# Fanchuana/OPUS-PLLM

Hardware: AMD Instinct MI355X
Metric: proteins_per_sec (higher is better)
Workload: dtype f16; 1 GPU; OPUS-PLLM-llama3_8b shape: batch 64/GPU, 512-residue proteins, 89-id prompt (+8 protein tokens = 96 positions), 32 new tokens, greedy (BASELINE configs[3] per-GPU shard: batch 512 over 8 GPUs); batch_per_gpu=64, residues=512, parallelism=replicas x1 (batch-sharded), all-gather of ids

## Files before the change

### opus-pllm_amd/csrc/api.cpp

```cpp
#include "../../include/opus_pllm.h"
#include "common.h"

#include <cmath>
#include <cstdarg>
#include <cstdio>
#include <cstdlib>
#include <cstring>
#include <algorithm>
#include <atomic>
#include <map>
#include <string>
#include <vector>

using namespace opus;

static thread_local char g_err[512] = "";
static int fail(int code, const char *fmt, ...) {
    va_list ap;
    va_start(ap, fmt);
    vsnprintf(g_err, sizeof(g_err), fmt, ap);
    va_end(ap);
    return code;
}
#define HIPC(expr)                                                                                   \
// ... 1023 lines not shown
        KL(KC_OTHER, 4.0 * M * F, launch_relu_h(c->d_act, (int64_t)M * F, s));
    }
    OPC(gemm(c, s, c->d_act, F, L.w2, M, H, F, L.b2, EPI_NONE, x, x, H, 1));
    return OPUS_OK;
}

static int lm_head_opt(opus_ctx *c, hipStream_t s, int B) {
    const opus_config &g = c->cfg;
    KL(KC_NORM, 6.0 * B * g.dec_dim, launch_layernorm(c->d_xl, c->dec_lnfw, c->dec_lnfb, g.dec_rms_eps, B, g.dec_dim, c->d_xln, nullptr, s));
    return gemm(c, s, c->d_xln, g.dec_dim, c->lm_head, B, g.dec_vocab, g.dec_dim, nullptr, EPI_NONE, nullptr, c->d_logits,
                g.dec_vocab, 1);
}

static int prefill_opt(opus_ctx *c, hipStream_t s, const half_t *embeds, const uint8_t *mask, int B, int T, bool all_rows,
                       const ContRows *cont) {
    const opus_config &g = c->cfg;
    const int H = g.dec_dim, M = B * T;
    HIPC(hipMemsetAsync(c->d_cnt, 0, HANDOFF_ERR * sizeof(int32_t), s));
    if (!cont) KL(KC_OTHER, 1.0 * M, launch_mask_to_kstart(mask, B, T, c->d_kstart, s));
    KL(KC_OTHER, 6.0 * M * H, launch_h2f(embeds, c->d_x, (int64_t)M * H, s));
    KL(KC_OTHER, 10.0 * M * H, launch_add_pos(c->d_x, c->dec_pos, cont ? cont->nkst : c->d_kstart, nullptr, 0, B, T, H, g.dec_max_pos + 1, s));
    for (int l = 0; l < g.dec_layers; ++l) OPC(opt_layer(c, s, c->dec[l], l, c->d_x, c->d_xn, M, B, T, false, cont));
    if (all_rows) return OPUS_OK;
    KL(KC_OTHER, 8.0 * B * H, launch_take_last(c->d_x, B, T, H, c->d_xl, s));
    OPC(lm_head_opt(c, s, B));
    OPC(reset_step(c, s, T));
    c->cur_B = B;
    c->cur_T = T;
    c->prefilled = true;
    return OPUS_OK;
}

static int decode_step_opt(opus_ctx *c, hipStream_t s) {
    const opus_config &g = c->cfg;
    const int B = c->cur_B, T = c->cur_T, H = g.dec_dim;
    KL(KC_OTHER, 10.0 * B * H, launch_add_pos(c->d_xl, c->dec_pos, c->d_kstart, c->d_step, -1, B, 1, H, g.dec_max_pos + 1, s));
    for (int l = 0; l < g.dec_layers; ++l) OPC(opt_layer(c, s, c->dec[l], l, c->d_xl, c->d_xln, B, B, T, true));
    OPC(lm_head_opt(c, s, B));
    KL(KC_OTHER, 8.0, launch_step_advance(c->d_step, s));
    return OPUS_OK;
}

static int prefill(opus_ctx *c, hipStream_t s, const half_t *embeds, const uint8_t *mask, int B, int T, bool all_rows = false,
                   const ContRows *cont = nullptr) {
    c->phase = cont ? PH_SCORE : PH_PREFILL;
    if (cont) {
        all_rows = true;
    } else {
        new_epoch(c);
        if (all_rows) {
            c->prefilled = false;
            c->cur_B = 0;
        }
    }
    if (c->cfg.dec_arch == 1) return prefill_opt(c, s, embeds, mask, B, T, all_rows, cont);
    const opus_config &g = c->cfg;
    const int H = g.dec_dim, F = g.dec_ffn, nh = g.dec_heads, nkv = g.dec_kv_heads, hd = g.dec_head_dim;
    const int QKV = (nh + 2 * nkv) * hd, QD = nh * hd;
    const int M = B * T;
    HIPC(hipMemsetAsync(c->d_cnt, 0, HANDOFF_ERR * sizeof(int32_t), s));
    if (!cont) KL(KC_OTHER, 1.0 * M, launch_mask_to_kstart(mask, B, T, c->d_kstart, s));
    KL(KC_OTHER, 6.0 * M * H, launch_h2f(embeds, c->d_x, (int64_t)M * H, s));
    static const bool no_ln_env = getenv("OPUS_NO_LN_FUSION") != nullptr;
    const bool no_ln_fusion = no_ln_env || g_knobs.no_ln_fusion;
    const bool qkv_pp = !no_ln_fusion && (H & 255) == 0 && (QKV & 255) == 0 && gemm_goes_pp(M, QKV);
    const bool gu_pp = !no_ln_fusion && (H & 255) == 0 && (F & 127) == 0 && gemm_goes_pp(M, 2 * F);
    bool have_stat = false, last_rows_done = false;
    auto finalize = [&]() -> int {
        KL(KC_NORM, 8.0 * M * (H / 64) + 8.0 * M, launch_ln_finalize(c->d_part, M, H / 64, H, g.dec_rms_eps, 1, c->d_stat, s));
        return OPUS_OK;
    };
    for (int l = 0; l < g.dec_layers; ++l) {
        const DecLayer &L = c->dec[l];
        if (have_stat && qkv_pp) {
            c->rq_ln_stat = c->d_stat;
            OPC(gemm(c, s, c->d_xn, H, L.wqkv, M, QKV, H, L.bqkv, EPI_NONE, nullptr, c->d_qkv, QKV, 0));
        } else {
            OPC(gemm_norm(c, s, c->d_x, g.dec_rms_eps, c->d_xn, L.wqkv, M, QKV, H, EPI_NONE, c->d_qkv, QKV, 0, L.bqkv));
        }
        if (cont) {
            KL(KC_OTHER, 4.0 * M * QKV, launch_dec_rope_cache(c->d_qkv, c->cs_dec, cont->nkst, B, T, nh, nkv, hd, nullptr, nullptr, 0, 0, s));
            OPC(attn_prefix(c, s, *cont, l, M));
        } else {
            KL(KC_OTHER, 4.0 * M * QKV,
               launch_dec_rope_cache(c->d_qkv, c->cs_dec, c->d_kstart, B, T, nh, nkv, hd, c->kc + l * c->cache_sl,
                                     c->vc + l * c->cache_sl, c->cache_sb, c->cache_sh, s));
            AttnParams a;
            a.Q = c->d_qkv; a.K = c->d_qkv + QD; a.V = c->d_qkv + QD + nkv * hd;
            a.q_sb = a.k_sb = a.v_sb = (int64_t)T * QKV;
            a.q_st = a.k_st = a.v_st = QKV;
            a.O = c->d_ctx; a.o_sb = (int64_t)T * QD; a.o_st = QD;
            a.kstart = c->d_kstart; a.kend = nullptr;
            a.B = B; a.T = T; a.heads = nh; a.group = nh / nkv; a.head_dim = hd; a.causal = 1;
            a.scale = 1.0f / sqrtf((float)hd);
            KLF(KC_ATTN_PREFILL, 2.0 * M * (QKV + QD), 2.0 * B * (double)T * T * QD, launch_attn_prefill(a, s));
        }
        if (l + 1 == g.dec_layers && T > 1 && !all_rows && !g_knobs.misc[7]) {
            half_t *ctx_last = c->d_qkv;
            KL(KC_OTHER, 4.0 * B * QD, launch_take_last(reinterpret_cast<const float *>(c->d_ctx), B, T, QD / 2, reinterpret_cast<float *>(ctx_last), s));
            KL(KC_OTHER, 8.0 * B * H, launch_take_last(c->d_x, B, T, H, c->d_xl, s));
            if (fuse_rows() && B <= 96) c->rq_xh = c->d_xln;
            OPC(gemm(c, s, ctx_last, QD, L.wo, B, H, QD, nullptr, EPI_NONE, c->d_xl, c->d_xl, H, 1));
            c->xh_src = c->rq_done ? c->d_xl : nullptr;
            OPC(gemm_norm(c, s, c->d_xl, g.dec_rms_eps, c->d_xln, L.wgu, B, 2 * F, H, EPI_SILU_GU16, c->d_act, F, 0));
            if (fuse_rows() && B <= 96) c->rq_xh = c->d_xln;
            OPC(gemm(c, s, c->d_act, F, L.wd, B, H, F, nullptr, EPI_NONE, c->d_xl, c->d_xl, H, 1));
            c->xh_src = c->rq_done ? c->d_xl : nullptr;
            c->xln_tiled = false;
            last_rows_done = true;
            break;
        }
        if (gu_pp) { c->rq_ln_part = c->d_part; c->rq_ln_xh = c->d_xn; }
        else if (fuse_rows() && M <= 96) c->rq_xh = c->d_xn;
        OPC(gemm(c, s, c->d_ctx, QD, L.wo, M, H, QD, nullptr, EPI_NONE, c->d_x, c->d_x, H, 1));
        c->xh_src = c->rq_done ? c->d_x : nullptr;
        have_stat = c->rq_ln_done != 0;
        if (have_stat) {
            OPC(finalize());
            c->rq_ln_stat = c->d_stat;
            OPC(gemm(c, s, c->d_xn, H, L.wgu, M, 2 * F, H, nullptr, EPI_SILU_GU16, nullptr, c->d_act, F, 0));
        } else {
            OPC(gemm_norm(c, s, c->d_x, g.dec_rms_eps, c->d_xn, L.wgu, M, 2 * F, H, EPI_SILU_GU16, c->d_act, F, 0));
        }
        if (qkv_pp && l + 1 < g.dec_layers) { c->rq_ln_part = c->d_part; c->rq_ln_xh = c->d_xn; }
        OPC(gemm(c, s, c->d_act, F, L.wd, M, H, F, nullptr, EPI_NONE, c->d_x, c->d_x, H, 1));
        have_stat = c->rq_ln_done != 0;
        if (have_stat) OPC(finalize());
    }
    if (all_rows) {
        c->xh_src = nullptr;
        return OPUS_OK;
    }
    if (!last_rows_done) {
        KL(KC_OTHER, 8.0 * B * H, launch_take_last(c->d_x, B, T, H, c->d_xl, s));
        c->xh_src = nullptr;
    }
    OPC(lm_head(c, s, B));
    OPC(reset_step(c, s, T));
    c->cur_B = B;
    c->cur_T = T;
    c->prefilled = true;
    return OPUS_OK;
}

static int decode_step(opus_ctx *c, hipStream_t s, const int32_t *d_tok) {
    c->phase = PH_DECODE;
    const opus_config &g = c->cfg;
    const int B = c->cur_B, T = c->cur_T;
    const int H = g.dec_dim, F = g.dec_ffn, nh = g.dec_heads, nkv = g.dec_kv_heads, hd = g.dec_head_dim;
    const int QKV = (nh + 2 * nkv) * hd, QD = nh * hd;
    const int ctx_cap = g.max_prompt + g.max_new_tokens;
    const bool rowscale = g.dec_arch == 0 && fuse_rows() && B > SKINNY_MAX_M && B <= MID_MAX_M && (H & 255) == 0;
    const bool qkv_tiled = rowscale && gemm_stream_would(B, QKV, H, 1, 1, 1, c->gemm_ws_bytes);
    const bool wo_tiled = rowscale && gemm_stream_would(B, H, QD, 0, 1, 0, c->gemm_ws_bytes);
    const bool down_tiled = rowscale && (F & 63) == 0 && gemm_stream_would(B, H, F, 0, 1, 0, c->gemm_ws_bytes);
    KL(KC_OTHER, 6.0 * B * H, launch_embed_tokens(d_tok, c->dec_emb, B, H, g.dec_vocab, c->d_xl, rowscale ? c->d_xln : nullptr,
                                                  rowscale ? c->d_ssq : nullptr, qkv_tiled ? 1 : 0, c->cs_dec, c->d_kstart, c->d_step, -1,
                                                  hd / 2, c->cs_row, c->d_cnt, HANDOFF_ERR, s));
    c->xln_tiled = qkv_tiled;
    c->xh_src = rowscale ? c->d_xl : nullptr;
    if (rowscale) c->ssq_nblk = H >> 8;
    if (g.dec_arch == 1) return decode_step_opt(c, s);
    for (int l = 0; l < g.dec_layers; ++l) {
        const DecLayer &L = c->dec[l];
        if (rowscale && c->xh_src == c->d_xl) {
            c->xh_src = nullptr;
            c->rq_force_wide = 1;
            c->rq_slab_only = 1;
            c->use_row_scale = true;
            c->row_eps = g.dec_rms_eps;
            c->rq_a_tiled = c->xln_tiled ? 1 : 0;
            OPC(gemm(c, s, c->d_xln, H, L.wqkv, B, QKV, H, L.bqkv, EPI_NONE, nullptr, c->d_qkv, QKV, 0));
            OPC(attn_decode(c, s, l, B, T, c->rq_ks > 1 ? c->rq_ks : 0, L.bqkv, wo_tiled ? 1 : 0));
        } else {
            OPC(gemm_norm(c, s, c->d_xl, g.dec_rms_eps, c->d_xln, L.wqkv, B, QKV, H, EPI_NONE, c->d_qkv, QKV, 0, L.bqkv));
            OPC(attn_decode(c, s, l, B, T, 0, nullptr, wo_tiled ? 1 : 0));
        }
        c->xln_tiled = false;
// ... 1169 lines not shown
    new_epoch(c);
    const int nkv = g.dec_kv_heads, hd = g.dec_head_dim, T0 = c->cur_T;
    for (int l = 0; l < g.dec_layers; ++l) {
        half_t *kc = c->kc + l * c->cache_sl, *vc = c->vc + l * c->cache_sl;
        KL(KC_OTHER, 8.0 * R * nkv * hd * T0, launch_kv_gather_rows(kc, c->kv_tmp, d_src_rows, R, (int64_t)row, nkv, c->cache_sh, c->d_step, T0, hd, 0, s));
        HIPC(launch_kv_gather_rows(vc, c->kv_tmp + layer, d_src_rows, R, (int64_t)row, nkv, c->cache_sh, c->d_step, T0, hd, 0, s));
        HIPC(launch_kv_gather_rows(kc, c->kv_tmp, d_src_rows, R, (int64_t)row, nkv, c->cache_sh, c->d_step, T0, hd, 1, s));
        HIPC(launch_kv_gather_rows(vc, c->kv_tmp + layer, d_src_rows, R, (int64_t)row, nkv, c->cache_sh, c->d_step, T0, hd, 1, s));
    }
    return OPUS_OK;
}

extern "C" int opus_last_logits(opus_ctx *c, float *d_out, int32_t B, void *stream) {
    if (!c || !d_out) return fail(OPUS_EBADARG, "last_logits: null pointer");
    if (!c->prefilled) return fail(OPUS_ESTATE, "last_logits before prefill");
    if (B < 1 || B > c->cur_B) return fail(OPUS_ESHAPE, "last_logits: B=%d but the last prefill had %d rows", B, c->cur_B);
    HIPC(hipSetDevice(c->device));
    HIPC(hipMemcpyAsync(d_out, c->d_logits, (size_t)B * c->cfg.dec_vocab * sizeof(float), hipMemcpyDeviceToDevice, (hipStream_t)stream));
    return OPUS_OK;
}

extern "C" int opus_debug_attention(opus_ctx *c, const void *Q, const void *K, const void *V, void *O,
                                    const int32_t *kstart, const int32_t *kend, int32_t B, int32_t T, int32_t heads,
                                    int32_t group, int32_t hd, int32_t causal, float scale, void *stream) {
    if (!c || !Q || !K || !V || !O) return fail(OPUS_EBADARG, "debug_attention: null pointer");
    if (B < 1 || T < 1 || heads < 1 || group < 1 || heads % group) return fail(OPUS_ESHAPE, "debug_attention: shape");
    HIPC(hipSetDevice(c->device));
    hipStream_t s = (hipStream_t)stream;
    AttnParams a;
    const int kvh = heads / group;
    a.Q = (const half_t *)Q; a.K = (const half_t *)K; a.V = (const half_t *)V; a.O = (half_t *)O;
    a.q_st = (int64_t)heads * hd; a.q_sb = a.q_st * T;
    a.k_st = a.v_st = (int64_t)kvh * hd; a.k_sb = a.v_sb = a.k_st * T;
    a.o_st = a.q_st; a.o_sb = a.q_sb;
    a.kstart = kstart; a.kend = kend; a.B = B; a.T = T; a.heads = heads; a.group = group; a.head_dim = hd;
    a.causal = causal; a.scale = scale;
    KLF(KC_ATTN_PREFILL, 2.0 * B * T * hd * (2.0 * heads + 2.0 * kvh), (causal ? 2.0 : 4.0) * B * (double)T * T * heads * hd,
        launch_attn_prefill(a, s));
    return OPUS_OK;
}

extern "C" int opus_debug_attn_decode(opus_ctx *c, const void *d_qkv, const void *d_k_hist, const void *d_v_hist,
                                      const int32_t *d_kstart, int32_t B, int32_t T0, int32_t step, void *d_out, void *d_k_new,
                                      void *d_v_new, void *stream) {
    if (!c || !d_qkv || !d_kstart || !d_out) return fail(OPUS_EBADARG, "debug_attn_decode: null pointer");
    const opus_config &g = c->cfg;
    const int L = T0 + step, nkv = g.dec_kv_heads, hd = g.dec_head_dim;
    if (B < 1 || B > g.max_batch || T0 < 1 || T0 > g.max_prompt || step < 0 || step >= g.max_new_tokens)
        return fail(OPUS_ESHAPE, "debug_attn_decode: B=%d T0=%d step=%d exceed the context (%d, %d, %d)", B, T0, step, g.max_batch,
                    g.max_prompt, g.max_new_tokens);
    if (L > 0 && (!d_k_hist || !d_v_hist)) return fail(OPUS_EBADARG, "debug_attn_decode: history is null");
    HIPC(hipSetDevice(c->device));
    hipStream_t s = (hipStream_t)stream;
    const size_t pitch = (size_t)c->cache_sh * sizeof(half_t), roww = (size_t)L * hd * sizeof(half_t);
    HIPC(hipMemcpy2DAsync(c->kc, pitch, d_k_hist, roww, roww, (size_t)B * nkv, hipMemcpyDeviceToDevice, s));
    HIPC(hipMemcpy2DAsync(c->vc, pitch, d_v_hist, roww, roww, (size_t)B * nkv, hipMemcpyDeviceToDevice, s));
    HIPC(hipMemcpyAsync(c->d_kstart, d_kstart, (size_t)B * sizeof(int32_t), hipMemcpyDeviceToDevice, s));
    OPC(reset_step(c, s, T0, step));
    HIPC(launch_embed_tokens(c->d_next, nullptr, B, 0, 1, c->d_xl, nullptr, nullptr, 0, c->cs_dec, c->d_kstart, c->d_step, -1, hd / 2,
                             c->cs_row, nullptr, 0, s));
    AttnDecodeParams a;
    a.qkv = (const half_t *)d_qkv; a.slabs = nullptr; a.ks = 0; a.slab_stride = 0; a.row_ssq = nullptr; a.row_nblk = 0; a.eps = 0.f; a.K = 0;
    a.bias = nullptr;
    a.cs_row = c->cs_row; a.kstart = c->d_kstart; a.step = c->d_step; a.T0 = -1; a.nh = g.dec_heads; a.nkv = nkv;
    a.kc = c->kc; a.vc = c->vc; a.cache_sb = c->cache_sb; a.cache_sh = c->cache_sh;
    a.ctx_cap = g.max_prompt + g.max_new_tokens; a.scale = 1.0f / sqrtf((float)hd); a.out = (half_t *)d_out; a.out_tiled = 0;
    c->phase = PH_DECODE;
    KL(KC_ATTN_DECODE, 4.0 * B * nkv * hd * (L + 1), launch_attn_decode(a, B, hd, s));
    const size_t one = (size_t)hd * sizeof(half_t);
    if (d_k_new) HIPC(hipMemcpy2DAsync(d_k_new, one, c->kc + (size_t)L * hd, pitch, one, (size_t)B * nkv, hipMemcpyDeviceToDevice, s));
    if (d_v_new) HIPC(hipMemcpy2DAsync(d_v_new, one, c->vc + (size_t)L * hd, pitch, one, (size_t)B * nkv, hipMemcpyDeviceToDevice, s));
    c->prefilled = false;
    new_epoch(c);
    return OPUS_OK;
}

extern "C" int opus_debug_knob(opus_ctx *c, const char *name, int32_t value) {
    if (!name) return fail(OPUS_EBADARG, "debug_knob: null name");
    if (c) drop_graphs(c);
    if (!strcmp(name, "no_stream")) g_knobs.no_stream = value;
    else if (!strcmp(name, "debug_a_tiled")) g_knobs.debug_a_tiled = value;
    else if (!strcmp(name, "no_ln_fusion")) g_knobs.no_ln_fusion = value;
    else if (!strcmp(name, "enc_full_last_layer")) g_knobs.enc_full_last_layer = value;
    else if (!strcmp(name, "poison_handoff")) {
        if (!c) return fail(OPUS_EBADARG, "poison_handoff needs a context");
        std::vector<int32_t> h(HANDOFF_ERR, 0);
        if (value) for (int i = 0; i < HANDOFF_ERR; ++i) h[i] = i < 512 ? value : ((i & 1) ? 0 : 1);
        HIPC(hipSetDevice(c->device));
        HIPC(hipDeviceSynchronize());
        HIPC(hipMemcpy(c->d_cnt, h.data(), h.size() * sizeof(int32_t), hipMemcpyHostToDevice));
    }
    else if (!strcmp(name, "pp_gm")) { if (value < 1 || value > 64) return fail(OPUS_EBADARG, "pp_gm out of range"); g_knobs.pp_gm = value; }
    else if (!strncmp(name, "misc", 4) && name[4] >= '0' && name[4] <= '7' && !name[5]) g_knobs.misc[name[4] - '0'] = value;
    else return fail(OPUS_EBADARG, "debug_knob: unknown knob '%s'", name);
    return OPUS_OK;
}

extern "C" int64_t opus_stat(opus_ctx *c, const char *name) {
    if (!c || !name) return -1;
    if (!strcmp(name, "graph_instantiations")) return c->graph_instantiations;
    if (!strcmp(name, "graph_replays")) return c->graph_replays;
    if (!strcmp(name, "graphs_cached")) return (int64_t)c->graphs.size();
    if (!strcmp(name, "decode_steps")) return c->decode_steps;
    return -1;
}

extern "C" int opus_timing_enable(opus_ctx *c, int32_t on) {
    if (!c) return fail(OPUS_EBADARG, "ctx is null");
    c->timing = on != 0;
    return OPUS_OK;
}
extern "C" int opus_timing_reset(opus_ctx *c) {
    if (!c) return fail(OPUS_EBADARG, "ctx is null");
    HIPC(hipDeviceSynchronize());
    timing_clear(c);
    return OPUS_OK;
}
static const char *kclass_names[KC_COUNT] = {"gemm_skinny", "gemm_mid", "gemm_wide", "gemm_ring", "gemm_pp", "gemm_tile", "splitk_reduce",
                                            "attn_prefill", "attn_decode", "norm", "other", "gemm_stream", "contact", "constraint", "logitproc",
                                            "xent"};
static const char *phase_names[PH_COUNT] = {"encode", "project", "splice", "prefill", "decode", "other", "score"};

extern "C" int opus_timing_get(opus_ctx *c, const char *kernel_class, const char *phase, double *ms, int64_t *launches,
                               double *bytes, double *flops) {
    if (!c || !kernel_class || !phase || !ms || !launches || !bytes || !flops) return fail(OPUS_EBADARG, "null argument");
    int k = -1, ph = -1;
    const bool any_k = !strcmp(kernel_class, "*"), any_p = !strcmp(phase, "*");
    for (int i = 0; i < KC_COUNT; ++i) if (!strcmp(kclass_names[i], kernel_class)) k = i;
    for (int i = 0; i < PH_COUNT; ++i) if (!strcmp(phase_names[i], phase)) ph = i;
    if (k < 0 && !any_k) return fail(OPUS_EBADARG, "unknown kernel class '%s'", kernel_class);
    if (ph < 0 && !any_p) return fail(OPUS_EBADARG, "unknown phase '%s'", phase);
    HIPC(hipDeviceSynchronize());
    double t = 0, b = 0, f = 0;
    int64_t n = 0;
    for (auto &r : c->recs) {
        if ((!any_k && r.klass != k) || (!any_p && r.phase != ph)) continue;
        float e = 0;
        HIPC(hipEventElapsedTime(&e, r.e0, r.e1));
        t += e;
        b += r.bytes;
        f += r.flops;
        ++n;
    }
    *ms = t;
    *launches = n;
    *bytes = b;
    *flops = f;
    return OPUS_OK;
}

extern "C" int opus_timing_names(char *buf, int32_t cap) {
    if (!buf || cap < 1) return fail(OPUS_EBADARG, "null buffer");
    std::string out;
    for (int i = 0; i < KC_COUNT; ++i) { out += kclass_names[i]; out += i + 1 < KC_COUNT ? "," : ";"; }
    for (int i = 0; i < PH_COUNT; ++i) { out += phase_names[i]; if (i + 1 < PH_COUNT) out += ","; }
    if ((int)out.size() + 1 > cap) return fail(OPUS_ESHAPE, "buffer too small (%zu needed)", out.size() + 1);
    memcpy(buf, out.c_str(), out.size() + 1);
    return OPUS_OK;
}
```

### opus-pllm_amd/csrc/attn_prefill.hip

```cpp
#include "common.h"
#include <type_traits>

namespace opus {

constexpr int KB = 64;

template <int HDP>
__device__ __forceinline__ int kswz(int row, int chunk) {
    if (HDP == 128) return chunk ^ (row & 15);
    if (HDP == 64) return chunk ^ ((row >> 1) & 7);
    return chunk;
}
template <int HD>
__device__ __forceinline__ int vswz(int row) {
    if (HD == 128) return (row & 7) << 1;
    if (HD == 64) return ((row >> 1) & 3) << 1;
    if (HD == 32) return ((row >> 2) & 1) << 1;
    return 0;
}

typedef float f2 __attribute__((ext_vector_type(2)));
__device__ __forceinline__ float max3(float a, float b, float c) {
    float r;
    asm("v_max3_f32 %0, %1, %2, %3" : "=v"(r) : "v"(a), "v"(b), "v"(c));
    return r;
}
__device__ __forceinline__ float xor16_max(float x) {
    float a = x, b = x, r;
    asm volatile("s_nop 1\n\tv_permlane16_swap_b32 %0, %1" : "+v"(a), "+v"(b));
    asm("v_max_f32 %0, %1, %2" : "=v"(r) : "v"(a), "v"(b));
    return r;
}
__device__ __forceinline__ void xor32_pair(float x, float &a, float &b) {
    a = x;
    b = x;
    asm volatile("s_nop 1\n\tv_permlane32_swap_b32 %0, %1" : "+v"(a), "+v"(b));
}

typedef short s4v __attribute__((ext_vector_type(4)));
typedef short s8v __attribute__((ext_vector_type(8)));

template <int HD, bool CAUSAL, int QT>
__global__ __launch_bounds__(256) void attn_prefill_kernel(AttnParams p) {
    constexpr int QW = 16 * QT, QB = 4 * QW;
    constexpr int HDP = HD < 32 ? 32 : HD;
    constexpr int KS = HDP / 32;
    constexpr int NO = HD / 16;
    constexpr int CH = HDP / 8;
    constexpr int VC = HD / 8;
    __shared__ __attribute__((aligned(16))) half_t sK[2][KB * HDP];
    __shared__ __attribute__((aligned(16))) half_t sV[2][KB * HD];

    const int tid = threadIdx.x, lane = tid & 63;
    const int wave = __builtin_amdgcn_readfirstlane(tid >> 6);
    const int g = lane >> 4, li = lane & 15;
    const int qtrim = (p.q_trim && p.cu) ? 1 : 0;
    const int nqb = (p.T - 2 * qtrim + QB - 1) / QB;
    const int id = blockIdx.x, slot = id >> 3;
    const int bh = (slot / nqb) * 8 + (id & 7);
    if (bh >= p.B * p.heads) return;
    const int b = bh / p.heads, h = bh % p.heads, hk = h / p.group;
    const int q0 = (slot % nqb) * QB + qtrim, qw = q0 + wave * QW;
    int T = p.T, Tq = p.T;
    int64_t qb_off = (int64_t)b * p.q_sb, kb_off = (int64_t)b * p.k_sb, vb_off = (int64_t)b * p.v_sb, ob_off = (int64_t)b * p.o_sb;
    if (p.cu) {
        const int r0 = p.cu[b];
        T = p.cu[b + 1] - r0;
        Tq = T - qtrim;
        if (q0 >= Tq) return;
        qb_off = (int64_t)r0 * p.q_st; kb_off = (int64_t)r0 * p.k_st; vb_off = (int64_t)r0 * p.v_st; ob_off = (int64_t)r0 * p.o_st;
    }
    const int kstart = (p.kstart && !p.cu) ? p.kstart[b] : 0;
    const int kend = (p.kend && !p.cu) ? p.kend[b] : T;

    const half_t *Qb = p.Q + qb_off + (int64_t)h * HD;
    const half_t *Kb = p.K + kb_off + (int64_t)hk * HD;
    const half_t *Vb = p.V + vb_off + (int64_t)hk * HD;

    h8 qf[QT][KS];
#pragma unroll
    for (int t = 0; t < QT; ++t) {
        int qr = qw + 16 * t + li;
        qr = qr < Tq ? qr : Tq - 1;
        const half_t *src = Qb + (int64_t)qr * p.q_st;
#pragma unroll
        for (int s = 0; s < KS; ++s) {
            const int d = 32 * s + 8 * g;
            qf[t][s] = d < HD ? *reinterpret_cast<const h8 *>(src + d) : h8{0, 0, 0, 0, 0, 0, 0, 0};
        }
    }
    f4 o[QT][NO];
    float mrow[QT], lrow[QT];
#pragma unroll
    for (int t = 0; t < QT; ++t) {
        mrow[t] = -INFINITY;
        lrow[t] = 0.f;
#pragma unroll
        for (int n = 0; n < NO; ++n) o[t][n] = f4{0.f, 0.f, 0.f, 0.f};
    }

    int k_lo = kstart / KB * KB;
    int k_hi = kend;
    if (CAUSAL) {
        const int last_q = (q0 + QB - 1 < T - 1 ? q0 + QB - 1 : T - 1);
        k_hi = k_hi < last_q + 1 ? k_hi : last_q + 1;
    }
    const float sc = p.scale * 1.4426950408889634f;
    const bool wave_live = qw < Tq;

    constexpr int KL = KB * CH / 256;
    constexpr int VN = KB * VC;
    constexpr int VL = VN >= 256 ? VN / 256 : 1;
    static_assert(KL >= 1, "tile too small for 256 threads");
    h8 kreg[KL], vreg[VL];
    const __amdgpu_buffer_rsrc_t krs = __builtin_amdgcn_make_buffer_rsrc((void *)Kb, 0, (int)(((int64_t)(T - 1) * p.k_st + HD) * 2), 0x00020000);
    const __amdgpu_buffer_rsrc_t vrs = __builtin_amdgcn_make_buffer_rsrc((void *)Vb, 0, (int)(((int64_t)(T - 1) * p.v_st + HD) * 2), 0x00020000);
    int koff[KL], voff[VL];
#pragma unroll
    for (int u = 0; u < KL; ++u) {
        const int i = tid + 256 * u, r = i / CH, c = i % CH;
        koff[u] = c * 8 < HD ? (int)((r * p.k_st + c * 8) * 2) : 0x7ffffff0;
    }
#pragma unroll
    for (int u = 0; u < VL; ++u) {
        const int i = tid + 256 * u, r = i / VC, c = i % VC;
        voff[u] = i < VN ? (int)((r * p.v_st + c * 8) * 2) : 0x7ffffff0;
    }
    auto load_tile = [&](int kt) {
        const int kb = kt * (int)p.k_st * 2, vb = kt * (int)p.v_st * 2;
#pragma unroll
        for (int u = 0; u < KL; ++u) kreg[u] = __builtin_bit_cast(h8, __builtin_amdgcn_raw_buffer_load_b128(krs, koff[u] + kb, 0, 0));
#pragma unroll
        for (int u = 0; u < VL; ++u) vreg[u] = __builtin_bit_cast(h8, __builtin_amdgcn_raw_buffer_load_b128(vrs, voff[u] + vb, 0, 0));
    };
    auto store_tile = [&](int buf) {
#pragma unroll
        for (int u = 0; u < KL; ++u) {
            const int i = tid + 256 * u, r = i / CH, c = i % CH;
            *reinterpret_cast<h8 *>(&sK[buf][r * HDP + kswz<HDP>(r, c) * 8]) = kreg[u];
        }
#pragma unroll
        for (int u = 0; u < VL; ++u) {
            const int i = tid + 256 * u, r = i / VC, c = i % VC;
            if (i < VN) *reinterpret_cast<h8 *>(&sV[buf][r * HD + (c ^ vswz<HD>(r)) * 8]) = vreg[u];
        }
    };

    if (k_lo < k_hi) {
        load_tile(k_lo);
        store_tile(0);
        if (k_lo + KB < k_hi) load_tile(k_lo + KB);
    }
    __syncthreads();
    auto tile_body = [&](auto nsub_tag, int kt, int buf) {
        {
            constexpr int NSUB = decltype(nsub_tag)::value, NJ = (NSUB + 1) / 2;
            const half_t *tK = sK[buf], *tV = sV[buf];
            f4 s[QT][4];
#pragma unroll
            for (int n = 0; n < NSUB; ++n) {
                const int r = 16 * n + li;
                h8 kf[KS];
#pragma unroll
                for (int ks = 0; ks < KS; ++ks) kf[ks] = *reinterpret_cast<const h8 *>(tK + r * HDP + kswz<HDP>(r, 4 * ks + g) * 8);
#pragma unroll
                for (int t = 0; t < QT; ++t) {
                    s[t][n] = f4{0.f, 0.f, 0.f, 0.f};
#pragma unroll
                    for (int ks = 0; ks < KS; ++ks) s[t][n] = mfma16(kf[ks], qf[t][ks], s[t][n]);
                }
            }
            const bool interior = kt >= kstart && kt + KB <= kend && (!CAUSAL || kt + KB - 1 <= qw);
            if (__builtin_expect(!interior, 0)) {
#pragma unroll
                for (int t = 0; t < QT; ++t) {
                    const int qi = qw + 16 * t + li;
#pragma unroll
                    for (int n = 0; n < NSUB; ++n)
#pragma unroll
                        for (int r = 0; r < 4; ++r) {
                            const int kj = kt + 16 * n + 4 * g + r;
                            bool vis = kj >= kstart && kj < kend;
                            if (CAUSAL) vis = vis && kj <= qi;
                            s[t][n][r] = vis ? s[t][n][r] : -INFINITY;
                        }
                }
            }
            h8 pf[QT][2];
#pragma unroll
            for (int t = 0; t < QT; ++t) {
                float mx = fmaxf(fmaxf(s[t][0][0], s[t][0][1]), fmaxf(s[t][0][2], s[t][0][3]));
#pragma unroll
                for (int n = 1; n < NSUB; ++n) mx = fmaxf(fmaxf(mx, fmaxf(s[t][n][0], s[t][n][1])), fmaxf(s[t][n][2], s[t][n][3]));
                float ma, mb;
                mx = xor16_max(mx);
                xor32_pair(mx, ma, mb);
                const float mnew = max3(mrow[t], ma, mb);
                const float msafe = mnew == -INFINITY ? 0.f : mnew;
                const float msc = msafe * sc;
                if (!__all(mnew == mrow[t])) {
                    const float alpha = __builtin_amdgcn_exp2f((mrow[t] - msafe) * sc);
                    lrow[t] *= alpha;
#pragma unroll
                    for (int n = 0; n < NO; ++n) o[t][n] *= alpha;
                    mrow[t] = mnew;
                }
                const f2 sc2 = f2{sc, sc}, msc2 = f2{msc, msc};
                f2 rs2 = f2{0.f, 0.f};
#pragma unroll
                for (int n = 0; n < NSUB; ++n)
#pragma unroll
                    for (int r = 0; r < 4; r += 2) {
                        const f2 a = f2{s[t][n][r], s[t][n][r + 1]} * sc2 - msc2;
                        const f2 e = f2{__builtin_amdgcn_exp2f(a[0]), __builtin_amdgcn_exp2f(a[1])};
                        s[t][n][r] = e[0];
                        s[t][n][r + 1] = e[1];
                        rs2 += e;
                    }
                lrow[t] += rs2[0] + rs2[1];
#pragma unroll
                for (int j = 0; j < NJ; ++j) {
                    const bool two = 2 * j + 1 < NSUB;
                    pf[t][j] = h8{(half_t)s[t][2 * j][0], (half_t)s[t][2 * j][1], (half_t)s[t][2 * j][2], (half_t)s[t][2 * j][3],
                                  two ? (half_t)s[t][two ? 2 * j + 1 : 0][0] : (half_t)0.f, two ? (half_t)s[t][two ? 2 * j + 1 : 0][1] : (half_t)0.f,
                                  two ? (half_t)s[t][two ? 2 * j + 1 : 0][2] : (half_t)0.f, two ? (half_t)s[t][two ? 2 * j + 1 : 0][3] : (half_t)0.f};
                }
            }
#pragma unroll
            for (int n = 0; n < NO; ++n)
#pragma unroll
                for (int j = 0; j < NJ; ++j) {
                    const int r0 = 16 * (2 * j) + 4 * g + (li >> 2), r1 = r0 + 16;
                    const int cc = 2 * n + ((li & 3) >> 1), off = (li & 1) * 4;
                    const s4v lo = __builtin_amdgcn_ds_read_tr16_b64_v4i16(
                        (__attribute__((address_space(3))) s4v *)(tV + r0 * HD + (cc ^ vswz<HD>(r0)) * 8 + off));
                    const s4v hi = __builtin_amdgcn_ds_read_tr16_b64_v4i16(
                        (__attribute__((address_space(3))) s4v *)(tV + r1 * HD + (cc ^ vswz<HD>(r1)) * 8 + off));
                    const s8v both = s8v{lo[0], lo[1], lo[2], lo[3], hi[0], hi[1], hi[2], hi[3]};
                    const h8 vf = __builtin_bit_cast(h8, both);
#pragma unroll
                    for (int t = 0; t < QT; ++t) o[t][n] = mfma16(vf, pf[t][j], o[t][n]);
                }
        }
    };
    auto run = [&](auto live_tag) {
        constexpr bool LIVE = decltype(live_tag)::value;
        int kt = k_lo, buf = 0;
        for (; k_hi - kt > 32; kt += KB, buf ^= 1) {
            if constexpr (LIVE) tile_body(std::integral_constant<int, 4>{}, kt, buf);
            if (kt + KB < k_hi) {
                store_tile(buf ^ 1);
                if (kt + 2 * KB < k_hi) load_tile(kt + 2 * KB);
            }
            __syncthreads();
        }
        if constexpr (LIVE) {
            if (kt < k_hi) {
                if (k_hi - kt > 16) tile_body(std::integral_constant<int, 2>{}, kt, buf);
                else tile_body(std::integral_constant<int, 1>{}, kt, buf);
            }
        }
    };
    if (wave_live) run(std::true_type{});
    else run(std::false_type{});

    if (!wave_live) return;
#pragma unroll
    for (int t = 0; t < QT; ++t) {
        float l = lrow[t];
        l += __shfl_xor(l, 16, 64);
        l += __shfl_xor(l, 32, 64);
        const int qi = qw + 16 * t + li;
        if (qi >= Tq) continue;
        const float inv = l > 0.f ? 1.0f / l : 0.f;
        half_t *dst = p.O + ob_off + (int64_t)qi * p.o_st + (int64_t)h * HD;
#pragma unroll
        for (int n = 0; n < NO; ++n)
            *reinterpret_cast<h4 *>(dst + 16 * n + 4 * g) =
                h4{(half_t)(o[t][n][0] * inv), (half_t)(o[t][n][1] * inv), (half_t)(o[t][n][2] * inv), (half_t)(o[t][n][3] * inv)};
    }
}

template <int HD, int QT>
static hipError_t launch_qt(const AttnParams &p, hipStream_t s) {
    const int nqb = cdiv(p.T - ((p.q_trim && p.cu) ? 2 : 0), 64 * QT);
    dim3 grid(((p.B * p.heads + 7) / 8) * 8 * nqb);
    if (p.causal) OPUS_LAUNCH(KC_ATTN_PREFILL, (attn_prefill_kernel<HD, true, QT>), grid, dim3(256), 0, s, p);
    else OPUS_LAUNCH(KC_ATTN_PREFILL, (attn_prefill_kernel<HD, false, QT>), grid, dim3(256), 0, s, p);
    return hipGetLastError();
}
template <int HD>
static hipError_t launch_hd(const AttnParams &p, hipStream_t s) {
    bool one = !(HD <= 64 && (int64_t)p.B * p.heads * cdiv(p.T, 128) >= 512);
    if (g_knobs.misc[3]) one = !one;
    return one ? launch_qt<HD, 1>(p, s) : launch_qt<HD, 2>(p, s);
}

hipError_t launch_attn_prefill(const AttnParams &p, hipStream_t s) {
    if (p.T <= 0 || p.B <= 0) return hipErrorInvalidValue;
    if ((p.o_st & 3) || (p.o_sb & 3) || (p.q_st & 7) || (p.k_st & 7) || (p.v_st & 7) || (p.q_sb & 7) || (p.k_sb & 7) || (p.v_sb & 7))
        return hipErrorInvalidValue;
    if ((int64_t)p.T * (p.k_st > p.v_st ? p.k_st : p.v_st) * 2 >= (1ll << 31)) return hipErrorInvalidValue;
    switch (p.head_dim) {
        case 16: return launch_hd<16>(p, s);
        case 32: return launch_hd<32>(p, s);
        case 64: return launch_hd<64>(p, s);
        case 128: return launch_hd<128>(p, s);
    }
    return hipErrorInvalidValue;
}

}
```

### opus-pllm_amd/csrc/common.h

```cpp
#pragma once
#include <hip/hip_runtime.h>
#include <hip/hip_ext.h>
#include <stdint.h>

namespace opus {

#ifdef OPUS_BF16
typedef __bf16 half_t;
typedef __bf16 h8 __attribute__((ext_vector_type(8)));
typedef __bf16 h4 __attribute__((ext_vector_type(4)));
typedef __bf16 h2 __attribute__((ext_vector_type(2)));
#else
typedef _Float16 half_t;
typedef _Float16 h8 __attribute__((ext_vector_type(8)));
typedef _Float16 h4 __attribute__((ext_vector_type(4)));
typedef _Float16 h2 __attribute__((ext_vector_type(2)));
#endif
typedef float f4 __attribute__((ext_vector_type(4)));
__device__ __forceinline__ f4 mfma16(h8 a, h8 b, f4 c) {
#ifdef OPUS_BF16
    return __builtin_amdgcn_mfma_f32_16x16x32_bf16(a, b, c, 0, 0, 0);
#else
    return __builtin_amdgcn_mfma_f32_16x16x32_f16(a, b, c, 0, 0, 0);
#endif
// ... 28 lines not shown
        if (ev_ && (klass) != ::opus::KC_REDUCE && !ev_->main_used) {                                                     \
            ev_->main_used = true;                                                                                        \
            ev_->main_class = (klass);                                                                                    \
            hipExtLaunchKernelGGL(kernel, grid, block, lds, stream, ev_->main0, ev_->main1, 0, __VA_ARGS__);              \
        } else if (ev_ && (klass) == ::opus::KC_REDUCE && !ev_->aux_used) {                                               \
            ev_->aux_used = true;                                                                                         \
            hipExtLaunchKernelGGL(kernel, grid, block, lds, stream, ev_->aux0, ev_->aux1, 0, __VA_ARGS__);                \
        } else {                                                                                                          \
            hipLaunchKernelGGL(kernel, grid, block, lds, stream, __VA_ARGS__);                                            \
        }                                                                                                                 \
    } while (0)
hipError_t ensure_dyn_lds(const void *fn, size_t bytes);

__device__ __forceinline__ void rotate_pair(float a, float b, float c, float sn, float &lo, float &hi) {
    lo = __builtin_fmaf(a, c, -__fmul_rn(b, sn));
    hi = __builtin_fmaf(b, c, __fmul_rn(a, sn));
    asm volatile("" : "+v"(lo), "+v"(hi));
}

__host__ __device__ __forceinline__ int64_t tiled_off(int row, int k, int K) {
    return ((int64_t)(row >> 4) * (K >> 6) + (k >> 6)) * 1024 + ((k & 63) >> 5) * 512 + ((((k & 31) >> 3) << 4) + (row & 15)) * 8 + (k & 7);
}

constexpr int HANDOFF_WORDS = 1024, HANDOFF_ERR = 1023;
constexpr int HANDOFF_SPIN_LIMIT = 1 << 19;

struct GemmParams {
    const half_t *A;
    const float *Af;
    float norm_eps;
    int64_t lda;
    const half_t *W;
    int M, N, K;
    const float *bias;
    const float *residual;
    int64_t ldr;
    void *C;
    int64_t ldc;
    int out_f32;
    int epi;
    float *ws;
    int64_t ws_bytes;
    half_t *xh_out;
    float *ssq_out;
    int *fused_done;
    const float *row_ssq;
    int row_nblk;
    int64_t ssq_cap = 0;
    int *nblk_out = nullptr;
    int slab_only = 0;
    int *ks_out = nullptr;
    int force_wide = 0;
    const float *rope_cs = nullptr;
    const int32_t *rope_pos = nullptr;
    int rope_T = 0, rope_cols = 0, rope_qcols = 0;
    float rope_qscale = 1.0f;
    int *rope_done = nullptr;
    int a_tiled = 0, xh_tiled = 0, c_tiled = 0;
    int *combine_cnt = nullptr;
    float *ln_part = nullptr;
    int *ln_done = nullptr;
    const float *ln_stat = nullptr;
    const float *ln_colsum = nullptr;
    int pp_gm = 8;
    int stagger = 0;
    int no_rot = 0;
    long long *trace = nullptr;
    int *pp_plan = nullptr;
};
constexpr int PP_PLAN_WORDS = 5;
enum PpTail { PP_TAIL_NONE = 0, PP_TAIL_PAIR = 1, PP_TAIL_REDUCE = 2 };

struct AttnParams {
    const half_t *Q, *K, *V;
    int64_t q_sb, q_st, k_sb, k_st, v_sb, v_st;
    half_t *O;
    int64_t o_sb, o_st;
    const int32_t *kstart;
    const int32_t *kend;
    int B, T, heads, group, head_dim, causal;
    float scale;
    const int32_t *cu = nullptr;
    int q_trim = 0;
};

hipError_t launch_gemm(const GemmParams &p, hipStream_t s, int *klass);
hipError_t launch_splitk_reduce(const GemmParams &p, int ks, hipStream_t s);
bool gemm_stream_ok(const GemmParams &p);
bool gemm_stream_would(int M, int N, int K, int slab_only, int a_tiled, int row_scale, int64_t ws_bytes);
hipError_t launch_gemm_stream(const GemmParams &p, hipStream_t s);
struct Knobs {
    int no_stream = 0;
    int no_ln_fusion = 0;
    int debug_a_tiled = 0;
    int pp_gm = 8;
    int enc_full_last_layer = 0;
    int misc[8] = {0, 0, 0, 0, 0, 0, 0, 0};
};
extern Knobs g_knobs;
template <int NWAVES, int ROWS>
__device__ __forceinline__ void block_row_rstd(const float *__restrict__ ssq, int M, int nblk, float inv_k, float eps, float *out,
                                               int wave, int lane) {
    constexpr int RW = (ROWS + NWAVES - 1) / NWAVES;
    float part[RW];
#pragma unroll
    for (int r = 0; r < RW; ++r) part[r] = 0.f;
    for (int j0 = 0; j0 < nblk; j0 += 256) {
        float t[RW][4];
#pragma unroll
        for (int r = 0; r < RW; ++r) {
            int row = wave + NWAVES * r;
            row = row < M ? row : M - 1;
#pragma unroll
            for (int u = 0; u < 4; ++u) {
                const int j = j0 + 64 * u + lane;
                t[r][u] = ssq[(int64_t)row * nblk + (j < nblk ? j : nblk - 1)];
                t[r][u] = j < nblk ? t[r][u] : 0.f;
            }
        }
#pragma unroll
        for (int r = 0; r < RW; ++r) part[r] += (t[r][0] + t[r][1]) + (t[r][2] + t[r][3]);
    }
#pragma unroll
    for (int r = 0; r < RW; ++r) {
        float q = part[r];
#pragma unroll
        for (int o = 32; o > 0; o >>= 1) q += __shfl_xor(q, o, 64);
        const int row = wave + NWAVES * r;
        if (lane == 0 && row < ROWS) out[row] = rsqrtf(q * inv_k + eps);
    }
}
bool gemm_goes_wide(int M, int N);
bool gemm_goes_pp(int M, int N);
hipError_t launch_attn_prefill(const AttnParams &p, hipStream_t s);
struct AttnPrefixParams {
    const half_t *kc, *vc;
    int64_t cache_sb, cache_sh;
    const int32_t *kstart;
    int Tp;
    const half_t *qkv;
    int n;
    const int32_t *list, *off, *blocks;
    half_t *out;
    int nh, nkv, hd;
    float scale;
    const int32_t *par = nullptr;
};
int attn_prefix_blocks(const int32_t *off, int P, int G, int n, int32_t *blocks);
int attn_prefix_max_blocks(int R, int P, int G, int n);
hipError_t launch_attn_prefix(const AttnPrefixParams &p, int nblocks, hipStream_t s);
hipError_t launch_attn_tree(const AttnPrefixParams &p, int nblocks, hipStream_t s);

struct ContactParams {
    const half_t *Q, *K;
    int64_t ld;
    const int32_t *cu;
    int B, heads;
    const float *w;
    float *A;
    int accumulate;
    float *rows;
    int64_t vld;
    int c0;
    float *part;
};
size_t contact_accum_lds(int heads);
hipError_t launch_esm_contact_accum(const ContactParams &p, int head_dim, int max_n, hipStream_t s);
hipError_t launch_esm_contact_colsum(const float *part, const int32_t *cu, int B, int heads, int max_n, float *vec, int64_t vld, int c0,
                                     int add, hipStream_t s);
hipError_t launch_esm_contact_scale(const float *vec, const int32_t *cu, int B, int C, const float *w, float *sw, hipStream_t s);
hipError_t launch_esm_contact_finish(const float *A, const float *vec, const float *sw, const int32_t *cu, int B, int C, int max_n,
                                     const float *bias, float *out, hipStream_t s);

hipError_t launch_layernorm(const float *x, const float *w, const float *b, float eps, int64_t rows, int D,
                            half_t *out_h, float *out_f, hipStream_t s);
hipError_t launch_ln_finalize(const float *part, int64_t rows, int nslab, int D, float eps, int rms, float *stat, hipStream_t s);
hipError_t launch_rmsnorm(const float *x, const float *w, float eps, int64_t rows, int D, half_t *out,
                          hipStream_t s);
hipError_t launch_l2norm(const float *x, int64_t rows, int D, half_t *out, hipStream_t s);
// ... 139 lines not shown
```

Measured before the change: 256.9 proteins/s.

## Fuse decoder prefill rotary and KV-cache write into attention kernel

Applies RoPE to Q and K tiles in registers inside the causal prefill attention kernel. One head per KV group writes the rotated K and the V rows into the KV cache, so the separate rope/cache kernel and its extra pass over QKV go away. On the last decoder layer only the final query block is computed, since only the last row's context is used. The cost is extra register pressure and cos/sin loads in the attention kernel, plus a serial pre-pass over the padded prefix for writer blocks.

```diff
diff --git a/opus-pllm_amd/csrc/api.cpp b/opus-pllm_amd/csrc/api.cpp
--- a/opus-pllm_amd/csrc/api.cpp
+++ b/opus-pllm_amd/csrc/api.cpp
@@ -1129,9 +1129,12 @@
             KL(KC_OTHER, 4.0 * M * QKV, launch_dec_rope_cache(c->d_qkv, c->cs_dec, cont->nkst, B, T, nh, nkv, hd, nullptr, nullptr, 0, 0, s));
             OPC(attn_prefix(c, s, *cont, l, M));
         } else {
-            KL(KC_OTHER, 4.0 * M * QKV,
-               launch_dec_rope_cache(c->d_qkv, c->cs_dec, c->d_kstart, B, T, nh, nkv, hd, c->kc + l * c->cache_sl,
-                                     c->vc + l * c->cache_sl, c->cache_sb, c->cache_sh, s));
+            const bool rope_fused = hd == 128 && nh % nkv == 0 && !g_knobs.no_prefill_rope_fusion;
+            const bool last_rows = l + 1 == g.dec_layers && T > 1 && !all_rows && !g_knobs.misc[7];
+            if (!rope_fused)
+                KL(KC_OTHER, 4.0 * M * QKV,
+                   launch_dec_rope_cache(c->d_qkv, c->cs_dec, c->d_kstart, B, T, nh, nkv, hd, c->kc + l * c->cache_sl,
+                                         c->vc + l * c->cache_sl, c->cache_sb, c->cache_sh, s));
             AttnParams a;
             a.Q = c->d_qkv; a.K = c->d_qkv + QD; a.V = c->d_qkv + QD + nkv * hd;
             a.q_sb = a.k_sb = a.v_sb = (int64_t)T * QKV;
@@ -1140,7 +1143,20 @@
             a.kstart = c->d_kstart; a.kend = nullptr;
             a.B = B; a.T = T; a.heads = nh; a.group = nh / nkv; a.head_dim = hd; a.causal = 1;
             a.scale = 1.0f / sqrtf((float)hd);
-            KLF(KC_ATTN_PREFILL, 2.0 * M * (QKV + QD), 2.0 * B * (double)T * T * QD, launch_attn_prefill(a, s));
+            double bytes = 2.0 * M * (QKV + QD), flops = 2.0 * B * (double)T * T * QD;
+            if (rope_fused) {
+                a.rope_cs = c->cs_dec;
+                a.kc = c->kc + l * c->cache_sl; a.vc = c->vc + l * c->cache_sl;
+                a.cache_sb = c->cache_sb; a.cache_sh = c->cache_sh;
+                a.q_last_block = last_rows ? 1 : 0;
+                bytes += 4.0 * M * nkv * hd;
+                if (last_rows) {
+                    const int tq = T - (T - 1) / 64 * 64;
+                    bytes = 2.0 * M * 2 * nkv * hd + 4.0 * B * tq * QD + 4.0 * M * nkv * hd;
+                    flops = 4.0 * B * (double)tq * T * QD;
+                }
+            }
+            KLF(KC_ATTN_PREFILL, bytes, flops, launch_attn_prefill(a, s));
         }
         if (l + 1 == g.dec_layers && T > 1 && !all_rows && !g_knobs.misc[7]) {
             half_t *ctx_last = c->d_qkv;
@@ -2476,6 +2492,7 @@
     else if (!strcmp(name, "debug_a_tiled")) g_knobs.debug_a_tiled = value;
     else if (!strcmp(name, "no_ln_fusion")) g_knobs.no_ln_fusion = value;
     else if (!strcmp(name, "enc_full_last_layer")) g_knobs.enc_full_last_layer = value;
+    else if (!strcmp(name, "no_prefill_rope_fusion")) g_knobs.no_prefill_rope_fusion = value;
     else if (!strcmp(name, "poison_handoff")) {
         if (!c) return fail(OPUS_EBADARG, "poison_handoff needs a context");
         std::vector<int32_t> h(HANDOFF_ERR, 0);
diff --git a/opus-pllm_amd/csrc/attn_prefill.hip b/opus-pllm_amd/csrc/attn_prefill.hip
--- a/opus-pllm_amd/csrc/attn_prefill.hip
+++ b/opus-pllm_amd/csrc/attn_prefill.hip
@@ -37,11 +37,26 @@
     asm volatile("s_nop 1\n\tv_permlane32_swap_b32 %0, %1" : "+v"(a), "+v"(b));
 }
 
+__device__ __forceinline__ void rope8_regs(h8 &lo, h8 &hi, const f4 (&cs)[4]) {
+    h8 olo, ohi;
+#pragma unroll
+    for (int j = 0; j < 8; ++j) {
+        const float c = cs[j >> 1][2 * (j & 1)], sn = cs[j >> 1][2 * (j & 1) + 1];
+        float rl, rh;
+        rotate_pair((float)lo[j], (float)hi[j], c, sn, rl, rh);
+        olo[j] = (half_t)rl;
+        ohi[j] = (half_t)rh;
+    }
+    lo = olo;
+    hi = ohi;
+}
+
 typedef short s4v __attribute__((ext_vector_type(4)));
 typedef short s8v __attribute__((ext_vector_type(8)));
 
-template <int HD, bool CAUSAL, int QT>
+template <int HD, bool CAUSAL, int QT, bool ROPE = false>
 __global__ __launch_bounds__(256) void attn_prefill_kernel(AttnParams p) {
+    static_assert(!ROPE || (HD == 128 && CAUSAL && QT == 1), "the fused rotary exists for the decoder prefill's instance only");
     constexpr int QW = 16 * QT, QB = 4 * QW;
     constexpr int HDP = HD < 32 ? 32 : HD;
     constexpr int KS = HDP / 32;
@@ -57,10 +72,12 @@
     const int qtrim = (p.q_trim && p.cu) ? 1 : 0;
     const int nqb = (p.T - 2 * qtrim + QB - 1) / QB;
     const int id = blockIdx.x, slot = id >> 3;
-    const int bh = (slot / nqb) * 8 + (id & 7);
+    const bool last_only = ROPE && p.q_last_block;
+    const int nqb_grid = last_only ? 1 : nqb;
+    const int bh = (slot / nqb_grid) * 8 + (id & 7);
     if (bh >= p.B * p.heads) return;
     const int b = bh / p.heads, h = bh % p.heads, hk = h / p.group;
-    const int q0 = (slot % nqb) * QB + qtrim, qw = q0 + wave * QW;
+    const int q0 = (last_only ? nqb - 1 : slot % nqb) * QB + qtrim, qw = q0 + wave * QW;
     int T = p.T, Tq = p.T;
     int64_t qb_off = (int64_t)b * p.q_sb, kb_off = (int64_t)b * p.k_sb, vb_off = (int64_t)b * p.v_sb, ob_off = (int64_t)b * p.o_sb;
     if (p.cu) {
@@ -78,6 +95,7 @@
     const half_t *Vb = p.V + vb_off + (int64_t)hk * HD;
 
     h8 qf[QT][KS];
+    auto load_q = [&]() {
 #pragma unroll
     for (int t = 0; t < QT; ++t) {
         int qr = qw + 16 * t + li;
@@ -88,7 +106,19 @@
             const int d = 32 * s + 8 * g;
             qf[t][s] = d < HD ? *reinterpret_cast<const h8 *>(src + d) : h8{0, 0, 0, 0, 0, 0, 0, 0};
         }
-    }
+        if constexpr (ROPE) {
+            const int pos = qr - kstart > 0 ? qr - kstart : 0;
+            const float *cs = p.rope_cs + (int64_t)pos * HD;
+#pragma unroll
+            for (int s = 0; s < KS / 2; ++s) {
+                const f4 *c4 = reinterpret_cast<const f4 *>(cs + (32 * s + 8 * g) * 2);
+                const f4 cv[4] = {c4[0], c4[1], c4[2], c4[3]};
+                rope8_regs(qf[t][s], qf[t][s + KS / 2], cv);
+            }
+        }
+    }
+    };
+    if constexpr (!ROPE) load_q();
     f4 o[QT][NO];
     float mrow[QT], lrow[QT];
 #pragma unroll
@@ -116,9 +146,31 @@
     const __amdgpu_buffer_rsrc_t krs = __builtin_amdgcn_make_buffer_rsrc((void *)Kb, 0, (int)(((int64_t)(T - 1) * p.k_st + HD) * 2), 0x00020000);
     const __amdgpu_buffer_rsrc_t vrs = __builtin_amdgcn_make_buffer_rsrc((void *)Vb, 0, (int)(((int64_t)(T - 1) * p.v_st + HD) * 2), 0x00020000);
     int koff[KL], voff[VL];
+    auto kmap = [&](int u, int &r, int &c) {
+        if constexpr (ROPE) {
+            const int i = tid + 256 * (u >> 1);
+            r = i / (CH / 2);
+            c = i % (CH / 2) + (CH / 2) * (u & 1);
+        } else {
+            const int i = tid + 256 * u;
+            r = i / CH;
+            c = i % CH;
+        }
+    };
+    const bool writer = ROPE && p.kc && h % p.group == 0 && q0 + QB >= T;
+    constexpr int KP = ROPE ? KL / 2 : 1;
+    f4 kcs[KP][4];
+    half_t *kcb = nullptr, *vcb = nullptr;
+    if constexpr (ROPE) {
+        if (writer) {
+            kcb = p.kc + (int64_t)b * p.cache_sb + (int64_t)hk * p.cache_sh;
+            vcb = p.vc + (int64_t)b * p.cache_sb + (int64_t)hk * p.cache_sh;
+        }
+    }
 #pragma unroll
     for (int u = 0; u < KL; ++u) {
-        const int i = tid + 256 * u, r = i / CH, c = i % CH;
+        int r, c;
+        kmap(u, r, c);
         koff[u] = c * 8 < HD ? (int)((r * p.k_st + c * 8) * 2) : 0x7ffffff0;
     }
 #pragma unroll
@@ -132,11 +184,45 @@
         for (int u = 0; u < KL; ++u) kreg[u] = __builtin_bit_cast(h8, __builtin_amdgcn_raw_buffer_load_b128(krs, koff[u] + kb, 0, 0));
 #pragma unroll
         for (int u = 0; u < VL; ++u) vreg[u] = __builtin_bit_cast(h8, __builtin_amdgcn_raw_buffer_load_b128(vrs, voff[u] + vb, 0, 0));
-    };
-    auto store_tile = [&](int buf) {
+        if constexpr (ROPE) {
+#pragma unroll
+            for (int j = 0; j < KP; ++j) {
+                int r, c;
+                kmap(2 * j, r, c);
+                int row = kt + r;
+                row = row < T ? row : T - 1;
+                const int pos = row - kstart > 0 ? row - kstart : 0;
+                const f4 *c4 = reinterpret_cast<const f4 *>(p.rope_cs + (int64_t)pos * HD + c * 16);
+#pragma unroll
+                for (int v = 0; v < 4; ++v) kcs[j][v] = c4[v];
+            }
+        }
+    };
+    auto rotate_tile = [&](int kt) {
+        if constexpr (ROPE) {
+#pragma unroll
+            for (int j = 0; j < KP; ++j) rope8_regs(kreg[2 * j], kreg[2 * j + 1], kcs[j]);
+            if (writer) {
+#pragma unroll
+                for (int u = 0; u < KL; ++u) {
+                    int r, c;
+                    kmap(u, r, c);
+                    if (kt + r < T) *reinterpret_cast<h8 *>(kcb + (int64_t)(kt + r) * HD + c * 8) = kreg[u];
+                }
+#pragma unroll
+                for (int u = 0; u < VL; ++u) {
+                    const int i = tid + 256 * u, r = i / VC, c = i % VC;
+                    if (i < VN && kt + r < T) *reinterpret_cast<h8 *>(vcb + (int64_t)(kt + r) * HD + c * 8) = vreg[u];
+                }
+            }
+        }
+    };
+    auto store_tile = [&](int buf, int kt) {
+        rotate_tile(kt);
 #pragma unroll
         for (int u = 0; u < KL; ++u) {
-            const int i = tid + 256 * u, r = i / CH, c = i % CH;
+            int r, c;
+            kmap(u, r, c);
             *reinterpret_cast<h8 *>(&sK[buf][r * HDP + kswz<HDP>(r, c) * 8]) = kreg[u];
         }
 #pragma unroll
@@ -146,10 +232,22 @@
         }
     };
 
+    if constexpr (ROPE) {
+        if (writer) {
+            const int pad_end = k_lo < T ? k_lo : T;
+            for (int kt = 0; kt < pad_end; kt += KB) {
+                load_tile(kt);
+                rotate_tile(kt);
+            }
+        }
+    }
     if (k_lo < k_hi) {
         load_tile(k_lo);
-        store_tile(0);
+        if constexpr (ROPE) load_q();
+        store_tile(0, k_lo);
         if (k_lo + KB < k_hi) load_tile(k_lo + KB);
+    } else if constexpr (ROPE) {
+        load_q();
     }
     __syncthreads();
     auto tile_body = [&](auto nsub_tag, int kt, int buf) {
@@ -249,7 +347,7 @@
         for (; k_hi - kt > 32; kt += KB, buf ^= 1) {
             if constexpr (LIVE) tile_body(std::integral_constant<int, 4>{}, kt, buf);
             if (kt + KB < k_hi) {
-                store_tile(buf ^ 1);
+                store_tile(buf ^ 1, kt + KB);
                 if (kt + 2 * KB < k_hi) load_tile(kt + 2 * KB);
             }
             __syncthreads();
@@ -285,6 +383,13 @@
 static hipError_t launch_qt(const AttnParams &p, hipStream_t s) {
     const int nqb = cdiv(p.T - ((p.q_trim && p.cu) ? 2 : 0), 64 * QT);
     dim3 grid(((p.B * p.heads + 7) / 8) * 8 * nqb);
+    if constexpr (HD == 128 && QT == 1) {
+        if (p.rope_cs) {
+            if (p.q_last_block) grid = dim3(((p.B * p.heads + 7) / 8) * 8);
+            OPUS_LAUNCH(KC_ATTN_PREFILL, (attn_prefill_kernel<HD, true, QT, true>), grid, dim3(256), 0, s, p);
+            return hipGetLastError();
+        }
+    }
     if (p.causal) OPUS_LAUNCH(KC_ATTN_PREFILL, (attn_prefill_kernel<HD, true, QT>), grid, dim3(256), 0, s, p);
     else OPUS_LAUNCH(KC_ATTN_PREFILL, (attn_prefill_kernel<HD, false, QT>), grid, dim3(256), 0, s, p);
     return hipGetLastError();
@@ -293,11 +398,16 @@
 static hipError_t launch_hd(const AttnParams &p, hipStream_t s) {
     bool one = !(HD <= 64 && (int64_t)p.B * p.heads * cdiv(p.T, 128) >= 512);
     if (g_knobs.misc[3]) one = !one;
+    if (p.rope_cs) one = true;
     return one ? launch_qt<HD, 1>(p, s) : launch_qt<HD, 2>(p, s);
 }
 
 hipError_t launch_attn_prefill(const AttnParams &p, hipStream_t s) {
     if (p.T <= 0 || p.B <= 0) return hipErrorInvalidValue;
+    if (p.rope_cs && (p.head_dim != 128 || !p.causal || p.cu || p.q_trim || p.kend || !p.kstart || p.heads % p.group ||
+                      (p.kc && (!p.vc || (p.cache_sb & 7) || (p.cache_sh & 7)))))
+        return hipErrorInvalidValue;
+    if (p.q_last_block && !p.rope_cs) return hipErrorInvalidValue;
     if ((p.o_st & 3) || (p.o_sb & 3) || (p.q_st & 7) || (p.k_st & 7) || (p.v_st & 7) || (p.q_sb & 7) || (p.k_sb & 7) || (p.v_sb & 7))
         return hipErrorInvalidValue;
     if ((int64_t)p.T * (p.k_st > p.v_st ? p.k_st : p.v_st) * 2 >= (1ll << 31)) return hipErrorInvalidValue;
diff --git a/opus-pllm_amd/csrc/common.h b/opus-pllm_amd/csrc/common.h
--- a/opus-pllm_amd/csrc/common.h
+++ b/opus-pllm_amd/csrc/common.h
@@ -134,6 +134,10 @@
     float scale;
     const int32_t *cu = nullptr;
     int q_trim = 0;
+    const float *rope_cs = nullptr;
+    half_t *kc = nullptr, *vc = nullptr;
+    int64_t cache_sb = 0, cache_sh = 0;
+    int q_last_block = 0;
 };
 
 hipError_t launch_gemm(const GemmParams &p, hipStream_t s, int *klass);
@@ -147,6 +151,7 @@
     int debug_a_tiled = 0;
     int pp_gm = 8;
     int enc_full_last_layer = 0;
+    int no_prefill_rope_fusion = 0;
     int misc[8] = {0, 0, 0, 0, 0, 0, 0, 0};
 };
 extern Knobs g_knobs;
```

New measurement: 257.3 proteins/s (median of 3 runs). No clear change (+0.2%).
